# liznerski/eoe

Measured on AMD Instinct MI355X. Metric: train images/sec, CLIP ViT-B/32 + HSC, 224x224, higher is better.
Workload: dtype fp16; 1 GPU; CLIP ViT-B/32 (12 layers) + Linear(512,256) + HSC, full fine-tune, Adam lr 1e-4 wd 1e-3, 224x224, 128 normal + 128 OE images per GPU per step; global_batch=256, parallelism=dp1, launch=eager, weight-gradient launches on a side stream under the dgrad chain, arithmetic=16-bit MFMA operands, fp32 accumulate

## Files before the change

### eoe_amd/_build.py

```python
import fcntl
import hashlib
import os
import shutil
import subprocess
import sys

HERE = os.path.dirname(os.path.abspath(__file__))
CSRC = os.path.join(HERE, "csrc")
INCLUDE = os.path.join(os.path.dirname(HERE), "include")
LIB = os.path.join(HERE, "libeoe_hip.so")
OBJDIR = os.path.join(HERE, "build")
SOURCES = ["api.cpp", "gemm.hip", "gemm_tn.hip", "elementwise.hip", "attention.hip", "conv.hip", "cbam.hip", "augment.hip",
           "vit.cpp", "parity.hip", "gemm256.hip", "comm.cpp", "gemm_tn256.hip", "gemm_w8.hip", "probe.hip",
           "msm.hip", "sharpen.hip", "clip_text.hip", "clip_text_driver.cpp", "normstats.hip", "evolve.hip", "curves.hip"]
CFLAGS = ["--offload-arch=gfx950", "-O3", "-std=c++17", "-fPIC", "-Wno-unused-value"]
EXTRA_CFLAGS = {"gemm_w8.hip": ["-mllvm", "-amdgpu-spill-vgpr-to-agpr=0"]}
LDFLAGS = ["--offload-arch=gfx950", "-shared", "-fPIC", "-Wl,--no-undefined"]


def hipcc_path():
    for cand in (shutil.which("hipcc"), "/opt/rocm/bin/hipcc"):
        if cand and os.path.exists(cand):
            return cand
    return None


def _sha(*chunks) -> str:
    h = hashlib.sha256()
    for c in chunks:
        h.update(c if isinstance(c, bytes) else str(c).encode())
        h.update(b"\0")
    return h.hexdigest()


def _read(path) -> bytes:
    with open(path, "rb") as f:
        return f.read()


def _headers_digest() -> str:
    hs = sorted(os.path.join(CSRC, f) for f in os.listdir(CSRC) if f.endswith((".h", ".hpp", ".inc")))
    hs += sorted(os.path.join(INCLUDE, f) for f in os.listdir(INCLUDE) if f.endswith(".h"))
    return _sha(*[_read(h) for h in hs])


def _flags(src: str = ""):
    return CFLAGS + EXTRA_CFLAGS.get(src, []) + (["-DEOE_AB"] if os.environ.get("EOE_AB") else []) + os.environ.get("EOE_CFLAGS", "").split()
# ... 88 lines not shown
```

### eoe_amd/_lib.py

```python
import ctypes as C
import os
import re

import torch

from . import _build

ABI_VERSION = 5
EOE_F16, EOE_BF16, EOE_F32 = 1, 2, 3
EOE_RESIZE_BILINEAR, EOE_RESIZE_BICUBIC = 2, 3
EOE_MSM_LPF, EOE_MSM_HPF, EOE_MSM_BLUR = 1, 2, 3
EOE_MSM_FORM_NONE, EOE_MSM_FORM_DENSE, EOE_MSM_FORM_RANK = 0, 1, 2
EOE_GCN_L1, EOE_GCN_L2 = 1, 2
EOE_COMM_I64, EOE_COMM_ID_BYTES, EOE_COMM_ALGO_RING, EOE_COMM_ALGO_RS_AG = 8, 128, 0, 1
EPI_NONE, EPI_GELU, EPI_RESIDUAL, EPI_GELU_BWD = 0, 1, 2, 3
ADAM_CHUNK, ADAM_GROUPS = 8192, 4
CHUNK_FP16 = 0x100
EOE_Y16 = 0x100

_vp, _i32, _i64, _f32, _sz = C.c_void_p, C.c_int32, C.c_int64, C.c_float, C.c_size_t


class ConvGeometry(C.Structure):
    _fields_ = [("n", _i32), ("H", _i32), ("W", _i32), ("C", _i32), ("kh", _i32), ("kw", _i32), ("stride", _i32), ("pad", _i32),
# ... 95 lines not shown
    _fields_ = [("f", VitBlockFwdArgs), ("dx_out", _vp), ("dx_in", _vp),
                ("g_ln1_g", _vp), ("g_ln1_b", _vp), ("g_ln2_g", _vp), ("g_ln2_b", _vp),
                ("g_b_in", _vp), ("g_b_out", _vp), ("g_b_fc", _vp), ("g_b_proj", _vp),
                ("g_w_in", _vp), ("g_w_out", _vp), ("g_w_fc", _vp), ("g_w_proj", _vp),
                ("accumulate", _i32),
                ("d16_a", _vp), ("d16_b", _vp), ("d16_c", _vp), ("dh", _vp), ("dqkv", _vp), ("dx_mid", _vp), ("red_scratch", _vp),
                ("tn_workspace", _vp), ("tn_workspace_bytes", _i64),
                ("next_d16", _vp), ("in_d16", _vp), ("in_red_scratch", _vp), ("async_wgrad", _i32), ("red_table", C.POINTER(RedTable))]


ALLREDUCE_FN = C.CFUNCTYPE(C.c_int, C.c_void_p, C.c_void_p, C.c_int64, C.c_int, C.c_void_p)

SIGNATURES = {
    "eoe_abi_version": [],
    "eoe_struct_size": [C.c_int],
    "eoe_last_error": [],
    "eoe_vit_side_join": [_vp],
    "eoe_red_table_flush": [C.POINTER(RedTable), _vp],
    "eoe_gemm_nt": [C.POINTER(GemmArgs), _vp],
    "eoe_gemm_tn": [C.POINTER(GemmArgs), _vp],
    "eoe_gemm_tn_grouped": [C.POINTER(GemmArgs), C.c_int, _vp],
    "eoe_cast_transpose": [_vp, _vp, _vp, C.c_int, C.c_int, C.c_int, _vp],
    "eoe_cast_transpose_multi": [_vp, C.c_int, C.c_int, _vp],
    "eoe_conv_pack_weight_multi": [_vp, C.c_int, C.c_int, _vp],
    "eoe_patchify": [_vp, _vp, _vp, _vp, C.c_int, C.c_int, C.c_int, C.c_int, _vp],
    "eoe_embed_lnpre_fwd": [_vp] * 8 + [C.c_int, C.c_int, C.c_int, _f32, _vp],
    "eoe_embed_lnpre_bwd": [_vp] * 10 + [C.c_int, C.c_int, C.c_int, C.c_int, _vp],
    "eoe_layernorm_fwd": [_vp, C.c_int, _vp, _vp, _vp, _vp, C.c_int, C.c_int, _f32, C.c_int, C.c_int, _vp],
    "eoe_layernorm_bwd": [_vp, C.c_int, _vp, C.c_int, _vp, _vp, _vp, _vp, C.c_int, _vp, _vp, _vp, _vp, _vp, C.c_int,
                          C.c_int, C.c_int, _vp],
    "eoe_linear_small_fwd": [_vp, _vp, _vp, _vp, C.c_int, C.c_int, C.c_int, _vp],
    "eoe_linear_small_bwd": [_vp, _vp, _vp, _vp, _vp, _vp, C.c_int, C.c_int, C.c_int, C.c_int, _vp],
    "eoe_zero_multi": [C.POINTER(_vp), C.POINTER(C.c_int), C.c_int, _vp],
    "eoe_cast_colsum": [_vp, _vp, _vp, _vp, C.c_int, C.c_int, C.c_int, C.c_int, _vp],
    "eoe_colsum": [_vp, C.c_int, _vp, C.c_int, C.c_int, C.c_int, C.c_int, _vp],
    "eoe_colsum_det": [_vp, C.c_int, _vp, _vp, C.c_int, C.c_int, C.c_int, _vp],
    "eoe_cast": [_vp, _vp, _sz, C.c_int, _vp],
    "eoe_attn_fwd": [_vp, _vp, C.c_int, C.c_int, C.c_int, C.c_int, _vp],
    "eoe_attn_bwd": [_vp, _vp, _vp, _vp, _vp, C.c_int, C.c_int, C.c_int, C.c_int, _vp],
    "eoe_attn_causal_fwd": [_vp, _vp, C.c_int, C.c_int, C.c_int, C.c_int, _vp],
    "eoe_clip_token_embed": [_vp, C.c_int, _vp, _vp, _vp, C.c_int, C.c_int, C.c_int, C.c_int, _vp],
    "eoe_clip_eot_ln": [_vp, _vp, C.c_int, _vp, _vp, _vp, C.c_int, C.c_int, C.c_int, _f32, C.c_int, _vp],
    "eoe_clip_text_fwd": [C.POINTER(ClipTextFwdArgs), _vp],
    "eoe_hsc_fwd": [_vp, _vp, _i64, _vp, _vp, _vp, _vp, C.c_int, C.c_int, _f32, _vp],
    "eoe_hsc_bwd": [_vp, _vp, _i64, _vp, _vp, _vp, C.c_int, C.c_int, _f32, C.c_int, _vp],
    "eoe_hsc_score": [_vp, _vp, C.c_int, C.c_int, _vp],
    "eoe_bce_fwd": [_vp, _vp, _i64, _vp, _vp, _vp, C.c_int, _f32, _vp],
    "eoe_bce_bwd": [_vp, _vp, _vp, _vp, C.c_int, _f32, _vp],
    "eoe_adam_tiles": [_vp, _vp, _vp, _vp, _vp, C.c_int, C.POINTER(AdamScalars), _f32, _f32, _f32, _f32, C.c_int, _vp, _vp],
    "eoe_adam_multi": [_vp, _vp, _vp, _vp, _vp, C.c_int, C.POINTER(AdamScalars), _f32, _f32, _f32, _f32, _vp, C.c_int,
                       _vp, _vp],
    "eoe_grads_nonfinite": [_vp, _vp, C.c_int, _vp, C.c_int, C.c_int, _vp],
    "eoe_vit_block_fwd": [C.POINTER(VitBlockFwdArgs), _vp],
    "eoe_vit_block_bwd": [C.POINTER(VitBlockBwdArgs), _vp],
    "eoe_im2col": [_vp, C.c_int, _vp, _vp, _vp] + [C.c_int] * 10 + [_vp],
    "eoe_col2im": [_vp, _vp] + [C.c_int] * 11 + [_vp],
    "eoe_conv_pack_weight": [_vp, _vp, _vp, _vp] + [C.c_int] * 7 + [_vp],
    "eoe_conv_unpack_wgrad": [_vp, _vp] + [C.c_int] * 8 + [_vp],
    "eoe_stem_pack_image": [_vp, _vp, _vp, _vp] + [C.c_int] * 8 + [_vp],
    "eoe_stem_pack_weight": [_vp, _vp] + [C.c_int] * 4 + [_vp],
    "eoe_stem_unpack_wgrad": [_vp, _vp] + [C.c_int] * 3 + [_vp],
    "eoe_bn_stats": [_vp, _vp, _vp, _vp, _vp, _vp, C.c_int, C.c_int, _f32, _f32, C.c_int, _vp],
    "eoe_bn_stats_partials": [_vp, C.c_int, _vp, _vp, _vp, _vp, _vp, C.c_int, C.c_int, _f32, _f32, _vp],
    "eoe_bn_act_pool_fwd": [_vp, _vp, _vp, _vp, _vp, _vp, C.c_int, C.c_int, C.c_int, C.c_int, C.c_int, C.c_int, C.c_int, _f32,
                            C.c_int, _vp],
    "eoe_colsum_f32": [_vp, _vp, _vp, C.c_int, C.c_int, C.c_int, _vp],
# ... 146 lines not shown
```

### eoe_amd/csrc/elementwise.hip

```cpp
#include "common.h"

namespace {

template <typename T>
__global__ __launch_bounds__(256) void cast_kernel(const float* __restrict__ src, T* __restrict__ dst, size_t n) {
    size_t i = ((size_t)blockIdx.x * blockDim.x + threadIdx.x) * 4;
    const size_t stride = (size_t)gridDim.x * blockDim.x * 4;
    for (; i + 3 < n; i += stride) {
        f32x4 v = *(const f32x4*)(src + i);
        *(u32x2*)(dst + i) = pack4<T>(v[0], v[1], v[2], v[3]);
    }
    if (blockIdx.x == 0 && threadIdx.x < (n & 3)) {
        size_t j = (n & ~(size_t)3) + threadIdx.x;
        dst[j] = (T)src[j];
    }
}

template <typename T>
__global__ __launch_bounds__(256) void cast_transpose_kernel(const float* __restrict__ src, T* __restrict__ dst, T* __restrict__ dst_t,
                                      int rows, int cols) {
    __shared__ float tile[64][65];
    const int c0 = blockIdx.x * 64, r0 = blockIdx.y * 64;
    const int tx = threadIdx.x & 63, ty = threadIdx.x >> 6;
    for (int r = ty; r < 64; r += 4) {
// ... 108 lines not shown
    const int c = blockIdx.x * 256 + cg * 4;
    float a[4] = {0.f, 0.f, 0.f, 0.f};
    if (c < cols) {
        for (int r = blockIdx.y * 4 + rl; r < rows; r += gridDim.y * 4) {
            const f32x4 v = *(const f32x4*)(x + (size_t)r * cols + c);
            *(u32x2*)(dst + (size_t)r * cols + c) = pack4<T>(v[0], v[1], v[2], v[3]);
#pragma unroll
            for (int k = 0; k < 4; ++k) a[k] += v[k];
        }
    }
#pragma unroll
    for (int k = 0; k < 4; ++k) red[rl][cg * 4 + k] = a[k];
    __syncthreads();
    const int cc = blockIdx.x * 256 + threadIdx.x;
    if (cc >= cols) return;
    const float t = (red[0][threadIdx.x] + red[1][threadIdx.x]) + (red[2][threadIdx.x] + red[3][threadIdx.x]);
    if (part) part[eoe_part_index(cc, blockIdx.y, gridDim.y, cols, blocked)] = t;
    else atomicAdd(out + cc, t);
}

struct ZeroArgs { float* p[EOE_ZERO_MAX]; int n[EOE_ZERO_MAX]; int count; };
__global__ __launch_bounds__(256) void zero_multi_kernel(ZeroArgs a) {
    const int b = blockIdx.y;
    if (b >= a.count) return;
    float* p = a.p[b];
    const int n = a.n[b];
    if ((((uintptr_t)p) & 15) == 0) {
        const int n4 = n >> 2;
        for (int i = blockIdx.x * blockDim.x + threadIdx.x; i < n4; i += gridDim.x * blockDim.x) ((f32x4*)p)[i] = (f32x4){0.f, 0.f, 0.f, 0.f};
        for (int i = (n4 << 2) + blockIdx.x * blockDim.x + threadIdx.x; i < n; i += gridDim.x * blockDim.x) p[i] = 0.f;
    } else {
        for (int i = blockIdx.x * blockDim.x + threadIdx.x; i < n; i += gridDim.x * blockDim.x) p[i] = 0.f;
    }
}

template <typename T>
__global__ __launch_bounds__(256) void patchify_kernel(const float* __restrict__ x, const float* __restrict__ mean,
                                const float* __restrict__ stdv, T* __restrict__ out, int res, int p) {
    const int g = res / p;
    const int n = blockIdx.x / g, py = blockIdx.x % g;
    const int kdim = 3 * p * p;
    float mu[3] = {0.f, 0.f, 0.f}, is[3] = {1.f, 1.f, 1.f};
    if (mean) {
#pragma unroll
        for (int c = 0; c < 3; ++c) { mu[c] = mean[c]; is[c] = 1.0f / stdv[c]; }
    }
    const int rq_row = res >> 2;
    const int nq = 3 * p * rq_row;
    const int sq = 256 / rq_row, rq = 256 - sq * rq_row;
    int i = threadIdx.x;
    int c = i / (p * rq_row), rem = i - c * (p * rq_row);
    int ky = rem / rq_row, xq = rem - ky * rq_row;
    const float* img = x + (size_t)n * 3 * res * res + (size_t)py * p * res;
    T* orow = out + (size_t)(n * g + py) * g * kdim;
    constexpr int U = 4;
    while (i < nq) {
        f32x4 v[U];
        int cc[U], oo[U];
#pragma unroll
        for (int u = 0; u < U; ++u) {
            const bool ok = i < nq;
            const int xx = xq * 4;
            v[u] = *(const f32x4*)(img + (ok ? ((size_t)c * res + ky) * res + xx : (size_t)0));
            const int px = xx / p, kx = xx - px * p;
            cc[u] = c;
            oo[u] = ok ? px * kdim + c * p * p + ky * p + kx : -1;
// ... 1243 lines not shown
    }
    if (dw) {
        if (!accumulate) {
            if (hipMemsetAsync(dw, 0, (size_t)N * K * sizeof(float), s) != hipSuccess ||
                (db && hipMemsetAsync(db, 0, (size_t)N * sizeof(float), s) != hipSuccess))
                return eoe_set_error(EOE_ERR_LAUNCH, "linear_small_bwd: memset failed");
        }
        int gy = cdiv(M, 32);
        if (gy > 64) gy = 64;
        hipLaunchKernelGGL(linear_small_dw_kernel, dim3(cdiv(K, 256), gy), dim3(256), 0, s, x, dy, dw, db, M, N, K);
        EOE_CHECK_LAUNCH("linear_small_dw");
    }
    return 0;
}

extern "C" int eoe_zero_multi(float* const* ptrs, const int* counts, int n, void* stream) {
    EOE_CHECK_ARG(ptrs && counts && n >= 1 && n <= EOE_ZERO_MAX, "zero_multi: n %d not in [1, %d]", n, EOE_ZERO_MAX);
    ZeroArgs a;
    int mx = 0;
    for (int i = 0; i < n; ++i) {
        EOE_CHECK_ARG(ptrs[i] && counts[i] >= 0, "zero_multi: bad buffer %d", i);
        a.p[i] = ptrs[i]; a.n[i] = counts[i];
        if (counts[i] > mx) mx = counts[i];
    }
    a.count = n;
    int gx = cdiv(mx, 1024);
    if (gx > 2048) gx = 2048;
    if (gx < 1) gx = 1;
    hipLaunchKernelGGL(zero_multi_kernel, dim3(gx, n), dim3(256), 0, (hipStream_t)stream, a);
    EOE_CHECK_LAUNCH("zero_multi");
    return 0;
}

extern "C" int eoe_cast_colsum(const float* x, void* dst, float* out, float* scratch, int rows, int cols, int dtype, int accumulate,
                               void* stream) {
    EOE_CHECK_ARG(x && dst && out && rows > 0 && cols > 0, "cast_colsum: bad args");
    EOE_CHECK_ARG(cols % 4 == 0, "cast_colsum: cols must be a multiple of 4");
    ProfScope ps("cast_colsum", 0, 6.0 * rows * cols, stream);
    int gy = cdiv(rows, 4 * 8);
    if (gy > EOE_CAST_COLSUM_PARTIALS) gy = EOE_CAST_COLSUM_PARTIALS;
    const bool deferred_mode = scratch && eoe_tls_defer;
    const int blocked = (cols & 63) == 0;
    if (!accumulate && !deferred_mode) {
        if (hipMemsetAsync(out, 0, (size_t)cols * sizeof(float), (hipStream_t)stream) != hipSuccess)
            return eoe_set_error(EOE_ERR_LAUNCH, "cast_colsum: memset failed");
    }
    DISPATCH_T(dtype, hipLaunchKernelGGL((cast_colsum_kernel<T>), dim3(cdiv(cols, 256), gy), dim3(256), 0,
                                         (hipStream_t)stream, x, (T*)dst, out, scratch, rows, cols, blocked));
    EOE_CHECK_LAUNCH("cast_colsum");
    if (scratch) EOE_TRY(eoe_finish_reduce(scratch, gy, cols, cols, out, nullptr, nullptr, blocked, stream));
    return 0;
}

extern "C" int eoe_hsc_fwd(const float* f, const int64_t* labels, int64_t nominal_label, float* loss, float* scores,
                           float* dists, float* losses, int n, int d, float inv_count, void* stream) {
    EOE_CHECK_ARG(f && labels && n > 0 && d > 0, "hsc_fwd: bad args");
    EOE_CHECK_ARG(!loss || losses, "hsc_fwd: the loss needs the per-sample `losses` buffer");
    hipLaunchKernelGGL(hsc_rows_kernel, dim3(cdiv(n, 4)), dim3(256), 0, (hipStream_t)stream, f, labels, nominal_label,
                       scores, dists, losses, n, d);
    EOE_CHECK_LAUNCH("hsc_rows");
    if (loss) {
        hipLaunchKernelGGL(sum_scale_kernel, dim3(1), dim3(256), 0, (hipStream_t)stream, losses, loss, n, inv_count);
        EOE_CHECK_LAUNCH("hsc_sum");
    }
    return 0;
}
// ... 200 lines not shown
```

### eoe_amd/csrc/gemm.hip

```cpp
#include "gemm_common.h"
#include <stdlib.h>
#include <map>
#include <mutex>
#include <type_traits>

unsigned long long* g_stamp_buf = nullptr;
extern int g_tn_flags;
extern int g_vit_side_stream;
extern int g_attn_flags;
extern int g_tn256_launches;
extern int g_parity_flags;
int eoe_launch_nt256(const void* gemm_p, int dtype, int epi, int mi, hipStream_t s);
bool eoe_w8_applies(const void* gemm_p, int epi);
int eoe_launch_w8(const void* gemm_p, int dtype, int epi, hipStream_t s);
bool eoe_w8_streamk(const void* gemm_p);

namespace {
extern int g_nt_flags;


template <typename T, int EPI, int NI, int FLAGS, int GATHER = 0>
__global__ __launch_bounds__(512, 2) void gemm_nt_kernel(GemmP p) {
    extern __shared__ __attribute__((aligned(16))) char smem[];
    const int tid = threadIdx.x, lane = tid & 63, wave = tid >> 6;
    constexpr int BNI = 32 * NI;
    const int tiles_n = (p.N + BNI - 1) / BNI;
    const int total_tiles = tiles_n * ((p.M + BM - 1) / BM);
    const int G = gridDim.x;
    const int my_tiles = (total_tiles - (int)blockIdx.x + G - 1) / G;
    const int nk = p.K / BK;
    const int iters = my_tiles * nk;

    __amdgpu_buffer_rsrc_t ra = make_rsrc(p.A, p.bytesA);
    __amdgpu_buffer_rsrc_t rb = make_rsrc(p.B, p.bytesB);

    unsigned offA[4], offB[2];
    int gh[4], gw[4];
    int gw3[4];
    int g_ky = 0, g_kx = 0, g_c0 = 0;
    int st_tile = 0, st_kt = 0, st_slot = 0;
    auto tile_origin = [&](int seq, int& m0, int& n0) {
        const int r = xcd_remap((int)blockIdx.x + seq * G, total_tiles);
        m0 = (r / tiles_n) * BM;
        n0 = (r % tiles_n) * BNI;
    };
    auto set_offsets = [&](int t) {
        int m0, n0;
// ... 641 lines not shown
    EOE_CHECK_LAUNCH("gemm_nt128");
    return finish_colsum(p, epi, MI, s);
}

template <typename T>
int launch_nt128w(const GemmP& p, int epi, hipStream_t s) {
    const int tiles = cdiv(p.M, 160) * cdiv(p.N, 256);
#define EOE_NT128W_CASE(E)                                                                  \
    case E:                                                                                 \
        { static bool once = (hipFuncSetAttribute((const void*)gemm_nt128w_kernel<T, E>, hipFuncAttributeMaxDynamicSharedMemorySize, SMEMW_BYTES), true); (void)once; } \
        hipLaunchKernelGGL((gemm_nt128w_kernel<T, E>), dim3(tiles), dim3(256), SMEMW_BYTES, s, p); \
        break;
    switch (epi) {
        EOE_NT128W_CASE(EOE_EPI_NONE)
        EOE_NT128W_CASE(EOE_EPI_GELU)
        EOE_NT128W_CASE(EOE_EPI_RESIDUAL)
        EOE_NT128W_CASE(EOE_EPI_GELU_BWD)
        default: return eoe_set_error(EOE_ERR_ARG, "gemm_nt: unknown epilogue %d", epi);
    }
#undef EOE_NT128W_CASE
    EOE_CHECK_LAUNCH("gemm_nt128w");
    return finish_colsum(p, epi, 5, s);
}

template <typename T>
int launch_nt128_auto(const GemmP& p, int epi, hipStream_t s) {
    const int slots = 2 * num_cus();
    const long t4 = (long)cdiv(p.M, 128) * cdiv(p.N, 128), t5 = (long)cdiv(p.M, 160) * cdiv(p.N, 128);
    const long c4 = (t4 + slots - 1) / slots * 128, c5 = (t5 + slots - 1) / slots * 160;
    const bool five = (g_nt_flags & 32) || (!(g_nt_flags & 16) && c5 <= c4);
    return five ? launch_nt128<T, 5>(p, epi, s) : launch_nt128<T, 4>(p, epi, s);
}

template <typename T>
__global__ __launch_bounds__(256) void nt_splitk_finish_kernel(const float* __restrict__ part, int S, int M, int N, float alpha,
                                                               const float* __restrict__ bias, const float* __restrict__ res, int ldres,
                                                               void* __restrict__ C, int ldc, int out_f32) {
    const int nq = N / 4;
    const int i = blockIdx.x * blockDim.x + threadIdx.x;
    if (i >= M * nq) return;
    const int m = i / nq, n = (i - m * nq) * 4;
    f32x4 v = *(const f32x4*)(part + (size_t)m * N + n);
    for (int s2 = 1; s2 < S; ++s2) v += *(const f32x4*)(part + ((size_t)s2 * M + m) * N + n);
    v *= alpha;
    if (bias) v += *(const f32x4*)(bias + n);
    if (res) v += *(const f32x4*)(res + (size_t)m * ldres + n);
    if (out_f32) *(f32x4*)((float*)C + (size_t)m * ldc + n) = v;
    else *(u32x2*)((T*)C + (size_t)m * ldc + n) = pack4<T>(v[0], v[1], v[2], v[3]);
}

template <typename T>
int launch_nt128_splitk(const GemmP& p, int epi, hipStream_t s) {
    const int nk = p.K / BK;
    if ((g_nt_flags & 8192) || !p.split_k || p.M > 1024 || nk < 24 || (epi != EOE_EPI_NONE && epi != EOE_EPI_RESIDUAL) || p.colsum || p.colsum_sq || p.accumulate ||
        (p.N & 15) || (p.ldc & 3) || (epi == EOE_EPI_RESIDUAL && (p.ldaux & 3)))
        return -1;
    int S = 8;
    while (S > 1 && (nk % S) != 0) S >>= 1;
    if (S < 2 || nk / S < 3) return -1;
    float* part = p.sk_part;
    if (!part || (size_t)S * p.M * p.N > (size_t)2 * num_cus() * 65536) return -1;
    GemmP q = p;
    q.C = part; q.ldc = p.N; q.out_f32 = 1; q.bias = nullptr; q.aux = nullptr; q.alpha = 1.0f;
    const int tiles = cdiv(p.M, 128) * cdiv(p.N, 128);
    { static bool once = (hipFuncSetAttribute((const void*)gemm_nt128_kernel<T, EOE_EPI_NONE, 4>, hipFuncAttributeMaxDynamicSharedMemorySize, smem128_bytes(4)), true); (void)once; }
    hipLaunchKernelGGL((gemm_nt128_kernel<T, EOE_EPI_NONE, 4>), dim3(tiles, S), dim3(256), smem128_bytes(4), s, q);
    EOE_CHECK_LAUNCH("gemm_nt128 (split k)");
    hipLaunchKernelGGL((nt_splitk_finish_kernel<T>), dim3(cdiv(p.M * (p.N / 4), 256)), dim3(256), 0, s, (const float*)part, S, p.M, p.N, p.alpha,
                       p.bias, epi == EOE_EPI_RESIDUAL ? (const float*)p.aux : nullptr, p.ldaux, p.C, p.ldc, p.out_f32);
    EOE_CHECK_LAUNCH("nt_splitk_finish");
    return 0;
}


int g_nt_flags = EOE_NT_DEFAULT_FLAGS;

template <typename T, int NI, int FLAGS>
int launch_nt_f(const GemmP& p, int epi, int grid, hipStream_t s) {
#define EOE_NT_CASE(E)                                                                      \
    case E:                                                                                 \
        { static bool once = (hipFuncSetAttribute((const void*)gemm_nt_kernel<T, E, NI, FLAGS>, hipFuncAttributeMaxDynamicSharedMemorySize, SMEM_BYTES), true); (void)once; } \
        hipLaunchKernelGGL((gemm_nt_kernel<T, E, NI, FLAGS>), dim3(grid), dim3(512), SMEM_BYTES, s, p); \
        break;
    switch (epi) {
        EOE_NT_CASE(EOE_EPI_NONE)
        EOE_NT_CASE(EOE_EPI_GELU)
        EOE_NT_CASE(EOE_EPI_RESIDUAL)
        EOE_NT_CASE(EOE_EPI_GELU_BWD)
        default: return eoe_set_error(EOE_ERR_ARG, "gemm_nt: unknown epilogue %d", epi);
    }
#undef EOE_NT_CASE
    EOE_CHECK_LAUNCH("gemm_nt");
    return finish_colsum(p, epi, 4, s);
}

template <typename T, int NI, int GATHER>
int launch_nt_conv(const GemmP& p, int grid, hipStream_t s) {
    static bool once = (hipFuncSetAttribute((const void*)gemm_nt_kernel<T, EOE_EPI_NONE, NI, EOE_NT_DEFAULT_FLAGS, GATHER>,
                                            hipFuncAttributeMaxDynamicSharedMemorySize, SMEM_BYTES), true);
    (void)once;
    hipLaunchKernelGGL((gemm_nt_kernel<T, EOE_EPI_NONE, NI, EOE_NT_DEFAULT_FLAGS, GATHER>), dim3(grid), dim3(512), SMEM_BYTES, s, p);
    EOE_CHECK_LAUNCH("gemm_nt");
    return finish_colsum(p, EOE_EPI_NONE, 4, s);
}

template <typename T, int NI>
int launch_nt_ni(const GemmP& p, int epi, int grid, hipStream_t s) {
#ifdef EOE_AB
    switch (g_nt_flags & 3) {
        case 0: return launch_nt_f<T, NI, 0>(p, epi, grid, s);
        case 1: return launch_nt_f<T, NI, 1>(p, epi, grid, s);
        case 2: return launch_nt_f<T, NI, 2>(p, epi, grid, s);
        default: return launch_nt_f<T, NI, 3>(p, epi, grid, s);
    }
#else
    return launch_nt_f<T, NI, EOE_NT_DEFAULT_FLAGS>(p, epi, grid, s);
#endif
}

template <typename T>
int launch_nt(const GemmP& p, int epi, int gather, hipStream_t s) {
    const int ncu = num_cus();
    if (epi == EOE_EPI_NONE && p.N <= 64 && (gather == 0 || gather == 1 || gather == 2) && !(g_nt_flags & 64)) {
        const int rc = gather == 2 ? launch_nt64<T, 2>(p, s) : (gather ? launch_nt64<T, 1>(p, s) : launch_nt64<T, 0>(p, s));
        return rc ? rc : finish_colsum(p, EOE_EPI_NONE, 4, s);
    }
    if (gather == 1 && epi == EOE_EPI_NONE && p.N >= 128 && !(g_nt_flags & 2048)) {
        const int slots = 2 * ncu;
        const long t4 = (long)cdiv(p.M, 128) * cdiv(p.N, 128), t5 = (long)cdiv(p.M, 160) * cdiv(p.N, 128);
        const long c4 = (t4 + slots - 1) / slots * 128, c5 = (t5 + slots - 1) / slots * 160;
        if (!p.colsum_sq && c5 < c4) return launch_nt128_gather<T, 5>(p, s);
        return launch_nt128_gather<T, 4>(p, s);
    }
    if (gather || (epi == EOE_EPI_NONE && p.N <= 64)) {
        const bool narrow = p.N <= 64;
        const int tiles = cdiv(p.M, BM) * cdiv(p.N, narrow ? 64 : 128);
        const int grid = tiles < ncu ? tiles : ncu;
        if (gather == 2) return narrow ? launch_nt_conv<T, 2, 2>(p, grid, s) : launch_nt_conv<T, 4, 2>(p, grid, s);
        if (gather == 3) return narrow ? launch_nt_conv<T, 2, 3>(p, grid, s) : launch_nt_conv<T, 4, 3>(p, grid, s);
        if (gather) return narrow ? launch_nt_conv<T, 2, 1>(p, grid, s) : launch_nt_conv<T, 4, 1>(p, grid, s);
        return launch_nt_conv<T, 2, 0>(p, grid, s);
    }
    if ((g_nt_flags & (128 | 256)) && epilogue_direct_ok(p, epi))
        return eoe_launch_nt256(&p, std::is_same<T, f16_t>::value ? EOE_F16 : EOE_BF16, epi, (g_nt_flags & 256) ? 8 : 5, s);
    const bool big = p.K >= 4096 && p.N >= 2048;
    if (gather == 0 && p.split_k) {
        const int rc = launch_nt128_splitk<T>(p, epi, s);
        if (rc >= 0) return rc;
    }
    if (!(g_nt_flags & (131072 | 4 | 8 | 512)) && gather == 0 && p.M >= 2048 && eoe_w8_applies(&p, epi)) {
        const long tiles = (long)cdiv(p.M, 256) * (p.N / 256);
        if ((g_nt_flags & 262144) || eoe_w8_streamk(&p) || tiles * 100 >= ((tiles + ncu - 1) / ncu) * ncu * 85) 
            return eoe_launch_w8(&p, std::is_same<T, f16_t>::value ? EOE_F16 : EOE_BF16, epi, s);
    }
    if (!(g_nt_flags & (4096 | 4 | 8 | 512)) && gather == 0 && !p.colsum_sq && (p.N % 256) == 0 && p.N >= 2048 && (p.K % 32) == 0 && p.M >= 2048) {
        const long tiles = (long)cdiv(p.M, 160) * (p.N / 256), slots = 2L * ncu;
        if (tiles * 10 >= ((tiles + slots - 1) / slots) * slots * 9) return launch_nt128w<T>(p, epi, s);
    }
    const bool gelu_wide = epi == EOE_EPI_GELU && p.N >= 2048 && p.K <= 1024 && !(g_nt_flags & 1024);
    if (((g_nt_flags & 512) || gelu_wide) && !(g_nt_flags & (4 | 8)) && epilogue_direct_ok(p, epi) && p.M >= 2048 && p.N >= 512) {
        const int nk = p.K / BK;
        long best = 0;
        int mi_best = 5;
        for (int mi : {5, 8}) {
            const long tiles = (long)cdiv(p.M, 32 * mi) * cdiv(p.N, 256);
            const long cost = ((tiles + ncu - 1) / ncu) * ((long)mi * (nk + 2) + 30);
            if (!best || cost < best) { best = cost; mi_best = mi; }
        }
        return eoe_launch_nt256(&p, std::is_same<T, f16_t>::value ? EOE_F16 : EOE_BF16, epi, mi_best, s);
    }
    if (big && !(g_nt_flags & (4 | 8)) && epilogue_direct_ok(p, epi) && p.M >= 2048)
        return eoe_launch_nt256(&p, std::is_same<T, f16_t>::value ? EOE_F16 : EOE_BF16, epi, 8, s);
    if (!p.colsum_sq && ((g_nt_flags & 8) || (!big && !(g_nt_flags & 4)))) return launch_nt128_auto<T>(p, epi, s);
    const int t4 = cdiv(p.M, BM) * cdiv(p.N, 128), t3 = cdiv(p.M, BM) * cdiv(p.N, 96);
    const int c4 = cdiv(t4, ncu) * 4, c3 = cdiv(t3, ncu) * 3;
    const int force = (g_nt_flags >> 4) & 7;
    const bool use3 = force ? (force == 3) : (c3 * 10 <= c4 * 9);
    const int tiles = use3 ? t3 : t4;
    const int grid = tiles < ncu ? tiles : ncu;
    return use3 ? launch_nt_ni<T, 3>(p, epi, grid, s) : launch_nt_ni<T, 4>(p, epi, grid, s);
// ... 135 lines not shown
```

### eoe_amd/csrc/vit.cpp

```cpp
#include "common.h"
#include <mutex>
#include <stdlib.h>

#define TRY(expr)                   \
    do {                            \
        int rc__ = (expr);          \
        if (rc__ != 0) return rc__; \
    } while (0)

extern int g_tn_flags;
bool eoe_tn_streamk_would_run(const eoe_gemm_args* args, int count, void* stream);
int eoe_red_table_append(eoe_red_table* t, EoeRedJobs* jobs, void* stream);
int g_vit_side_stream = 1;

namespace {

struct SideStream {
    hipStream_t s = nullptr;
    hipEvent_t fork = nullptr, join = nullptr, wgrad_done[2] = {nullptr, nullptr};
    bool ok = false;
    unsigned seq = 0;
    bool recorded[2] = {false, false};
};
SideStream* side_stream(hipStream_t main) {
// ... 96 lines not shown
    } guard(b->red_scratch ? &jobs : nullptr);
    float* red_fc = b->red_scratch;
    float* red_ln2 = red_fc ? red_fc + (size_t)((M + 63) / 64) * H : nullptr;
    float* red_attn = red_fc ? red_ln2 + EOE_LN_SCRATCH(D) : nullptr;
    float* red_ln1 = red_fc ? red_attn + (size_t)a->n * 3 * D : nullptr;
    float* red_cast = red_fc ? red_ln1 + EOE_LN_SCRATCH(D) : nullptr;
    eoe_gemm_args g, w[4];
    const bool handed = !cls && b->in_d16 && b->in_red_scratch && b->red_scratch && b->in_red_scratch != b->red_scratch;
    const void* dy_proj = handed ? b->in_d16 : b->d16_a;
    if (handed) {
        const float* in_ln1 = b->in_red_scratch + (size_t)((M + 63) / 64) * H + EOE_LN_SCRATCH(D) + (size_t)a->n * 3 * D;
        int rows = (M + 7) / 8;
        if (rows > EOE_LN_PARTIALS) rows = EOE_LN_PARTIALS;
        if (!eoe_defer_reduce(in_ln1, rows, 3 * D, D, nullptr, nullptr, b->g_b_proj, 1))
            return eoe_set_error(EOE_ERR_ARG, "vit_block_bwd: could not queue the handed-over column sums");
    } else {
        TRY(eoe_cast_colsum(b->dx_out, b->d16_a, b->g_b_proj, red_cast, Mo, D, dt, 1, stream));
    }
    g = gemm(a, dy_proj, a->w_proj_t, b->dh, nullptr, Mo, H, D, D, D, H, dt);
    g.epilogue = EOE_EPI_GELU_BWD; g.aux = a->hpre; g.ldaux = H;
    if (b->red_scratch) {
        g.colsum = b->g_b_fc; g.workspace = red_fc; g.workspace_bytes = (int64_t)EOE_NT_COLSUM_WORKSPACE_BYTES(Mo, H);
        TRY(eoe_gemm_nt(&g, stream));
    } else {
        TRY(eoe_gemm_nt(&g, stream));
        TRY(eoe_colsum(b->dh, H, b->g_b_fc, Mo, H, dt, 1, stream));
    }
    g = gemm(a, b->dh, a->w_fc_t, b->d16_b, nullptr, Mo, D, H, H, H, D, dt);
    g.split_k = cls ? 1 : 0;
    TRY(eoe_gemm_nt(&g, stream));
    float* dx_mid_o = cls ? (float*)((char*)b->d16_a + (((size_t)Mo * D * 2 + 255) & ~(size_t)255)) : b->dx_mid;
    TRY(eoe_layernorm_bwd(b->d16_b, 0, a->x_mid, D, a->stats2, a->ln2_g, b->dx_out, dx_mid_o, D, b->d16_c, b->g_ln2_g,
                          b->g_ln2_b, b->g_b_out, red_ln2, Mo, D, dt, stream));
    if (cls) {
        if (hipMemsetAsync(b->dx_mid, 0, (size_t)M * D * sizeof(float), s) != hipSuccess ||
            hipMemcpy2DAsync(b->dx_mid, (size_t)ldrow * sizeof(float), dx_mid_o, (size_t)D * sizeof(float), (size_t)D * sizeof(float), Mo,
                             hipMemcpyDeviceToDevice, s) != hipSuccess ||
            hipMemsetAsync(b->d16_b, 0, (size_t)M * D * 2, s) != hipSuccess)
            return eoe_set_error(EOE_ERR_LAUNCH, "vit_block_bwd: zero-fill / scatter of the class-token rows failed");
    }
    g = gemm(a, b->d16_c, a->w_out_t, b->d16_b, nullptr, Mo, D, D, D, D, ldrow, dt);
    TRY(eoe_gemm_nt(&g, stream));
    TRY(eoe_attn_bwd(a->qkv, b->d16_b, b->dqkv, red_attn ? b->g_b_in : nullptr, red_attn, a->n, a->L, a->heads, dt, stream));
    g = gemm(a, b->dqkv, a->w_in_t, b->d16_b, nullptr, M, D, 3 * D, 3 * D, 3 * D, D, dt);
    TRY(eoe_gemm_nt(&g, stream));
    if (!b->red_scratch) TRY(eoe_colsum(b->dqkv, 3 * D, b->g_b_in, M, 3 * D, dt, 1, stream));
    w[0] = gemm(b->dh, a->xn2, b->g_w_fc, nullptr, H, D, Mo, H, D, D, dt);
    w[1] = gemm(dy_proj, a->hact, b->g_w_proj, nullptr, D, H, Mo, D, H, H, dt);
    w[2] = gemm(b->dqkv, a->xn1, b->g_w_in, nullptr, 3 * D, D, M, 3 * D, D, D, dt);
    w[3] = gemm(b->d16_c, a->att, b->g_w_out, nullptr, D, D, Mo, D, ldrow, D, dt);
    for (int i = 0; i < 4; ++i) { w[i].out_f32 = 1; w[i].accumulate = acc; }
    w[0].workspace = b->tn_workspace; w[0].workspace_bytes = b->tn_workspace ? b->tn_workspace_bytes : 0;
    eoe_gemm_args wc[3] = {w[0], w[1], w[3]};
    w[2].workspace = cls ? w[0].workspace : nullptr; w[2].workspace_bytes = cls ? w[0].workspace_bytes : 0;
    auto launch_wgrads = [&](void* st) -> int {
        if (!cls) return eoe_gemm_tn_grouped(w, 4, st);
        TRY(eoe_gemm_tn_grouped(wc, 3, st));
        return eoe_gemm_tn_grouped(&w[2], 1, st);
    };
    const bool streamk = !cls && eoe_tn_streamk_would_run(w, 4, stream);
    SideStream* ss = (g_vit_side_stream == 2 || (g_vit_side_stream && (!streamk || b->async_wgrad))) && b->red_scratch ? side_stream(s) : nullptr;
    if (ss && b->async_wgrad) {
        const unsigned e_prev = (ss->seq + 1) & 1, e_old = ss->seq & 1;
        if (ss->recorded[e_old]) {
            if (hipStreamWaitEvent(s, ss->wgrad_done[e_old], 0) != hipSuccess) return eoe_set_error(EOE_ERR_LAUNCH, "vit_block_bwd: stream wait failed");
            ss->recorded[e_old] = false;
        }
        if (b->async_wgrad < 2 && ss->recorded[e_prev]) {
            if (hipStreamWaitEvent(s, ss->wgrad_done[e_prev], 0) != hipSuccess) return eoe_set_error(EOE_ERR_LAUNCH, "vit_block_bwd: stream wait failed");
            ss->recorded[e_prev] = false;
        }
        if (hipEventRecord(ss->fork, s) != hipSuccess || hipStreamWaitEvent(ss->s, ss->fork, 0) != hipSuccess)
            return eoe_set_error(EOE_ERR_LAUNCH, "vit_block_bwd: fork failed");
// ... 40 lines not shown
```

### include/eoe_hip.h

```cpp
#ifndef EOE_HIP_H
#define EOE_HIP_H

#include <stddef.h>
#include <stdint.h>

#ifdef __cplusplus
extern "C" {
#endif

#define EOE_ABI_VERSION 5

enum { EOE_OK = 0, EOE_ERR_ARG = 1, EOE_ERR_LAUNCH = 2, EOE_ERR_UNSUPPORTED = 3 };
enum { EOE_F16 = 1, EOE_BF16 = 2, EOE_F32 = 3  };

int eoe_abi_version(void);
int eoe_struct_size(int which);
const char* eoe_last_error(void);

enum {
    EOE_EPI_NONE = 0,
    EOE_EPI_GELU = 1,
    EOE_EPI_RESIDUAL = 2,
    EOE_EPI_GELU_BWD = 3
};
// ... 52 lines not shown
int eoe_patchify(const float* x, const float* mean, const float* std, void* out, int n, int res, int patch,
                 int dtype, void* stream);

int eoe_embed_lnpre_fwd(const float* tok, const float* cls, const float* pos, const float* gamma,
                        const float* beta, float* x0, float* y, float* stats, int n, int L, int D, float eps,
                        void* stream);
int eoe_embed_lnpre_bwd(const float* dy, const float* x0, const float* stats, const float* gamma, void* dtok,
                        float* dcls, float* dpos, float* dgamma, float* dbeta, float* scratch, int n, int L, int D, int dtype,
                        void* stream);

int eoe_layernorm_fwd(const float* x, int ldx, const float* gamma, const float* beta, void* y, float* stats,
                      int rows, int D, float eps, int dtype, int out_f32, void* stream);
#define EOE_LN_PARTIALS 512
#define EOE_LN_SCRATCH(D) ((size_t)EOE_LN_PARTIALS * 3 * (D))
int eoe_layernorm_bwd(const void* dy, int dy_f32, const float* x, int ldx, const float* stats,
                      const float* gamma, const float* dres, float* dx_out, int ld_out, void* dx16,
                      float* dgamma, float* dbeta, float* dxsum, float* red_scratch, int rows, int D, int dtype,
                      void* stream);

int eoe_colsum(const void* x, int ldx, float* out, int rows, int cols, int dtype, int accumulate, void* stream);
#define EOE_COLSUM_PARTIALS 256
int eoe_colsum_det(const void* x, int ldx, float* out, float* scratch, int rows, int cols, int dtype, void* stream);

#define EOE_CAST_COLSUM_PARTIALS 256
int eoe_cast_colsum(const float* x, void* dst, float* out, float* scratch, int rows, int cols, int dtype, int accumulate, void* stream);

int eoe_linear_small_fwd(const float* x, const float* w, const float* bias, float* y, int M, int N, int K, void* stream);
int eoe_linear_small_bwd(const float* x, const float* w, const float* dy, float* dx, float* dw, float* db, int M, int N,
                         int K, int accumulate, void* stream);

#define EOE_ZERO_MAX 12
int eoe_zero_multi(float* const* ptrs, const int* counts, int n, void* stream);

int eoe_cast(const float* src, void* dst, size_t n, int dtype, void* stream);

int eoe_attn_fwd(const void* qkv, void* out, int n, int L, int heads, int dtype, void* stream);
int eoe_attn_bwd(const void* qkv, const void* dout, void* dqkv, float* dbias, float* bias_scratch, int n, int L, int heads,
                 int dtype, void* stream);

int eoe_attn_causal_fwd(const void* qkv, void* out, int n, int L, int heads, int dtype, void* stream);
int eoe_clip_token_embed(const void* tok, int tok_i64, const float* token_embedding, const float* positional_embedding, float* out, int n,
                         int L, int D, int vocab, void* stream);
int eoe_clip_eot_ln(const float* x, const void* tok, int tok_i64, const float* gamma, const float* beta, void* y, int n, int L, int D,
                    float eps, int dtype, void* stream);
typedef struct {
    int32_t n, L, D, heads, layers, vocab, embed_dim, dtype;
    float eps;
    int32_t tok_i64;
    const void* tokens;
    const float* token_embedding;
    const float* positional_embedding;
    const float* const* ln1_g; const float* const* ln1_b; const float* const* ln2_g; const float* const* ln2_b;
    const float* const* b_in; const float* const* b_out; const float* const* b_fc; const float* const* b_proj;
    const void* const* w_in; const void* const* w_out; const void* const* w_fc; const void* const* w_proj;
    const float *lnf_g, *lnf_b;
    const void* proj_t;
    float *x0, *x1;
    void *xn, *qkv, *att, *hact;
    float* stats;
    void* eot16;
    float* out;
    void* nt_sk_workspace;
    int64_t nt_sk_workspace_bytes;
} eoe_clip_text_fwd_args;
int eoe_clip_text_fwd(const eoe_clip_text_fwd_args* args, void* stream);

// ... 339 lines not shown
```

Before: 25570 images/sec.

## Add small-M rows GEMM kernel and fuse class-token scatter and zero-fill

Measured after the change: 25690 images/sec, median of 6. About the same (+0.5%).

```diff
diff --git a/eoe_amd/_build.py b/eoe_amd/_build.py
--- a/eoe_amd/_build.py
+++ b/eoe_amd/_build.py
@@ -12,7 +12,7 @@
 OBJDIR = os.path.join(HERE, "build")
 SOURCES = ["api.cpp", "gemm.hip", "gemm_tn.hip", "elementwise.hip", "attention.hip", "conv.hip", "cbam.hip", "augment.hip",
            "vit.cpp", "parity.hip", "gemm256.hip", "comm.cpp", "gemm_tn256.hip", "gemm_w8.hip", "probe.hip",
-           "msm.hip", "sharpen.hip", "clip_text.hip", "clip_text_driver.cpp", "normstats.hip", "evolve.hip", "curves.hip"]
+           "msm.hip", "sharpen.hip", "clip_text.hip", "clip_text_driver.cpp", "normstats.hip", "evolve.hip", "curves.hip", "gemm_rows.hip"]
 CFLAGS = ["--offload-arch=gfx950", "-O3", "-std=c++17", "-fPIC", "-Wno-unused-value"]
 EXTRA_CFLAGS = {"gemm_w8.hip": ["-mllvm", "-amdgpu-spill-vgpr-to-agpr=0"]}
 LDFLAGS = ["--offload-arch=gfx950", "-shared", "-fPIC", "-Wl,--no-undefined"]
diff --git a/eoe_amd/_lib.py b/eoe_amd/_lib.py
--- a/eoe_amd/_lib.py
+++ b/eoe_amd/_lib.py
@@ -151,6 +151,7 @@
     "eoe_linear_small_fwd": [_vp, _vp, _vp, _vp, C.c_int, C.c_int, C.c_int, _vp],
     "eoe_linear_small_bwd": [_vp, _vp, _vp, _vp, _vp, _vp, C.c_int, C.c_int, C.c_int, C.c_int, _vp],
     "eoe_zero_multi": [C.POINTER(_vp), C.POINTER(C.c_int), C.c_int, _vp],
+    "eoe_cls_scatter_fill": [_vp, _vp, _vp, C.c_int, C.c_int, C.c_int, _vp],
     "eoe_cast_colsum": [_vp, _vp, _vp, _vp, C.c_int, C.c_int, C.c_int, C.c_int, _vp],
     "eoe_colsum": [_vp, C.c_int, _vp, C.c_int, C.c_int, C.c_int, C.c_int, _vp],
     "eoe_colsum_det": [_vp, C.c_int, _vp, _vp, C.c_int, C.c_int, C.c_int, _vp],
diff --git a/eoe_amd/csrc/elementwise.hip b/eoe_amd/csrc/elementwise.hip
--- a/eoe_amd/csrc/elementwise.hip
+++ b/eoe_amd/csrc/elementwise.hip
@@ -164,6 +164,20 @@
     } else {
         for (int i = blockIdx.x * blockDim.x + threadIdx.x; i < n; i += gridDim.x * blockDim.x) p[i] = 0.f;
     }
+}
+
+__global__ __launch_bounds__(256) void cls_scatter_fill_kernel(f32x4* __restrict__ dx_mid, const f32x4* __restrict__ dx_cls,
+                                                               u32x4* __restrict__ d16, unsigned n4, unsigned n8, FDiv q, FDiv L) {
+    const unsigned stride = gridDim.x * blockDim.x, t = blockIdx.x * blockDim.x + threadIdx.x;
+    for (unsigned i = t; i < n4; i += stride) {
+        unsigned row, c, img, l;
+        q.divmod(i, row, c);
+        L.divmod(row, img, l);
+        f32x4 v = {0.f, 0.f, 0.f, 0.f};
+        if (l == 0) v = dx_cls[img * q.d + c];
+        dx_mid[i] = v;
+    }
+    for (unsigned i = t; i < n8; i += stride) d16[i] = (u32x4){0u, 0u, 0u, 0u};
 }
 
 template <typename T>
@@ -1473,6 +1487,19 @@
     return 0;
 }
 
+extern "C" int eoe_cls_scatter_fill(float* dx_mid, const float* dx_cls, void* d16, int n, int L, int D, void* stream) {
+    EOE_CHECK_ARG(dx_mid && dx_cls && d16 && n > 0 && L > 0 && D > 0 && (D % 8) == 0, "cls_scatter_fill: bad args (D must be a multiple of 8)");
+    EOE_CHECK_ARG(((((uintptr_t)dx_mid) | ((uintptr_t)dx_cls) | ((uintptr_t)d16)) & 15) == 0, "cls_scatter_fill: buffers must be 16-byte aligned");
+    const long long n4 = (long long)n * L * (D / 4);
+    EOE_CHECK_ARG(n4 < 0x7fffffffll, "cls_scatter_fill: %d x %d x %d is too large", n, L, D);
+    int gx = (int)((n4 + 255) / 256);
+    if (gx > 2048) gx = 2048;
+    hipLaunchKernelGGL(cls_scatter_fill_kernel, dim3(gx), dim3(256), 0, (hipStream_t)stream, (f32x4*)dx_mid, (const f32x4*)dx_cls, (u32x4*)d16,
+                       (unsigned)n4, (unsigned)(n4 / 2), FDiv((unsigned)(D / 4)), FDiv((unsigned)L));
+    EOE_CHECK_LAUNCH("cls_scatter_fill");
+    return 0;
+}
+
 extern "C" int eoe_cast_colsum(const float* x, void* dst, float* out, float* scratch, int rows, int cols, int dtype, int accumulate,
                                void* stream) {
     EOE_CHECK_ARG(x && dst && out && rows > 0 && cols > 0, "cast_colsum: bad args");
diff --git a/eoe_amd/csrc/gemm.hip b/eoe_amd/csrc/gemm.hip
--- a/eoe_amd/csrc/gemm.hip
+++ b/eoe_amd/csrc/gemm.hip
@@ -1,4 +1,5 @@
 #include "gemm_common.h"
+#include "gemm_rows_plan.h"
 #include <stdlib.h>
 #include <map>
 #include <mutex>
@@ -13,6 +14,7 @@
 int eoe_launch_nt256(const void* gemm_p, int dtype, int epi, int mi, hipStream_t s);
 bool eoe_w8_applies(const void* gemm_p, int epi);
 int eoe_launch_w8(const void* gemm_p, int dtype, int epi, hipStream_t s);
+int eoe_launch_nt_rows(const void* gemm_p, int dtype, int epi, int splits, hipStream_t s);
 bool eoe_w8_streamk(const void* gemm_p);
 
 namespace {
@@ -720,6 +722,14 @@
     return five ? launch_nt128<T, 5>(p, epi, s) : launch_nt128<T, 4>(p, epi, s);
 }
 
+static EoeNtPlanIn plan_in(const GemmP& p, int epi, int gather) {
+    EoeNtPlanIn q;
+    q.M = p.M; q.N = p.N; q.K = p.K; q.epi = epi; q.split_k = p.split_k; q.flags = g_nt_flags; q.gather = gather;
+    q.colsum = p.colsum != nullptr; q.colsum_sq = p.colsum_sq; q.accumulate = p.accumulate; q.ldc = p.ldc; q.ldaux = p.ldaux;
+    q.part_floats = p.sk_part ? (long long)2 * num_cus() * 65536 : 0;
+    return q;
+}
+
 template <typename T>
 __global__ __launch_bounds__(256) void nt_splitk_finish_kernel(const float* __restrict__ part, int S, int M, int N, float alpha,
                                                                const float* __restrict__ bias, const float* __restrict__ res, int ldres,
@@ -738,22 +748,20 @@
 }
 
 template <typename T>
-int launch_nt128_splitk(const GemmP& p, int epi, hipStream_t s) {
-    const int nk = p.K / BK;
-    if ((g_nt_flags & 8192) || !p.split_k || p.M > 1024 || nk < 24 || (epi != EOE_EPI_NONE && epi != EOE_EPI_RESIDUAL) || p.colsum || p.colsum_sq || p.accumulate ||
-        (p.N & 15) || (p.ldc & 3) || (epi == EOE_EPI_RESIDUAL && (p.ldaux & 3)))
-        return -1;
-    int S = 8;
-    while (S > 1 && (nk % S) != 0) S >>= 1;
-    if (S < 2 || nk / S < 3) return -1;
+int launch_nt128_splitk(const GemmP& p, int epi, bool rows, hipStream_t s) {
+    const int S = eoe_nt_splits(plan_in(p, epi, 0));
+    if (S < 2) return -1;
     float* part = p.sk_part;
-    if (!part || (size_t)S * p.M * p.N > (size_t)2 * num_cus() * 65536) return -1;
     GemmP q = p;
     q.C = part; q.ldc = p.N; q.out_f32 = 1; q.bias = nullptr; q.aux = nullptr; q.alpha = 1.0f;
-    const int tiles = cdiv(p.M, 128) * cdiv(p.N, 128);
-    { static bool once = (hipFuncSetAttribute((const void*)gemm_nt128_kernel<T, EOE_EPI_NONE, 4>, hipFuncAttributeMaxDynamicSharedMemorySize, smem128_bytes(4)), true); (void)once; }
-    hipLaunchKernelGGL((gemm_nt128_kernel<T, EOE_EPI_NONE, 4>), dim3(tiles, S), dim3(256), smem128_bytes(4), s, q);
-    EOE_CHECK_LAUNCH("gemm_nt128 (split k)");
+    if (rows) {
+        EOE_TRY(eoe_launch_nt_rows(&q, std::is_same<T, f16_t>::value ? EOE_F16 : EOE_BF16, EOE_EPI_NONE, S, s));
+    } else {
+        const int tiles = cdiv(p.M, 128) * cdiv(p.N, 128);
+        { static bool once = (hipFuncSetAttribute((const void*)gemm_nt128_kernel<T, EOE_EPI_NONE, 4>, hipFuncAttributeMaxDynamicSharedMemorySize, smem128_bytes(4)), true); (void)once; }
+        hipLaunchKernelGGL((gemm_nt128_kernel<T, EOE_EPI_NONE, 4>), dim3(tiles, S), dim3(256), smem128_bytes(4), s, q);
+        EOE_CHECK_LAUNCH("gemm_nt128 (split k)");
+    }
     hipLaunchKernelGGL((nt_splitk_finish_kernel<T>), dim3(cdiv(p.M * (p.N / 4), 256)), dim3(256), 0, s, (const float*)part, S, p.M, p.N, p.alpha,
                        p.bias, epi == EOE_EPI_RESIDUAL ? (const float*)p.aux : nullptr, p.ldaux, p.C, p.ldc, p.out_f32);
     EOE_CHECK_LAUNCH("nt_splitk_finish");
@@ -809,6 +817,10 @@
 template <typename T>
 int launch_nt(const GemmP& p, int epi, int gather, hipStream_t s) {
     const int ncu = num_cus();
+    if (eoe_nt_rows_applies(plan_in(p, epi, gather))) {
+        const int rc = launch_nt128_splitk<T>(p, epi, true, s);
+        return rc >= 0 ? rc : eoe_launch_nt_rows(&p, std::is_same<T, f16_t>::value ? EOE_F16 : EOE_BF16, epi, 1, s);
+    }
     if (epi == EOE_EPI_NONE && p.N <= 64 && (gather == 0 || gather == 1 || gather == 2) && !(g_nt_flags & 64)) {
         const int rc = gather == 2 ? launch_nt64<T, 2>(p, s) : (gather ? launch_nt64<T, 1>(p, s) : launch_nt64<T, 0>(p, s));
         return rc ? rc : finish_colsum(p, EOE_EPI_NONE, 4, s);
@@ -833,7 +845,7 @@
         return eoe_launch_nt256(&p, std::is_same<T, f16_t>::value ? EOE_F16 : EOE_BF16, epi, (g_nt_flags & 256) ? 8 : 5, s);
     const bool big = p.K >= 4096 && p.N >= 2048;
     if (gather == 0 && p.split_k) {
-        const int rc = launch_nt128_splitk<T>(p, epi, s);
+        const int rc = launch_nt128_splitk<T>(p, epi, false, s);
         if (rc >= 0) return rc;
     }
     if (!(g_nt_flags & (131072 | 4 | 8 | 512)) && gather == 0 && p.M >= 2048 && eoe_w8_applies(&p, epi)) {
diff --git a/eoe_amd/csrc/gemm_rows.hip b/eoe_amd/csrc/gemm_rows.hip
--- /dev/null
+++ b/eoe_amd/csrc/gemm_rows.hip
@@ -0,0 +1,114 @@
+#include "gemm_common.h"
+
+namespace {
+
+constexpr int ROWS_TILE = 64;
+constexpr int ROWS_SLOTS = 8;
+constexpr int ROWS_HALF_BYTES = ROWS_TILE * BK * 2;
+constexpr int ROWS_SLOT_BYTES = 2 * ROWS_HALF_BYTES;
+constexpr int ROWS_SMEM_BYTES = ROWS_SLOTS * ROWS_SLOT_BYTES;
+static_assert(ROWS_SLOTS == 8, "the counted wait below is 4 * (ROWS_SLOTS - 2) = 24 and the slot index is masked with 7");
+
+template <typename T, int EPI>
+__global__ __launch_bounds__(256, 1) void gemm_rows_kernel(GemmP p) {
+    extern __shared__ __attribute__((aligned(16))) char smem[];
+    constexpr int MI = 4, NI = 1;
+    const int tid = threadIdx.x, lane = tid & 63, wave = tid >> 6;
+    const int tiles_n = (p.N + ROWS_TILE - 1) / ROWS_TILE;
+    const int mt = (int)blockIdx.x / tiles_n, nt = (int)blockIdx.x - mt * tiles_n;
+    const int m0 = mt * ROWS_TILE, n0 = nt * ROWS_TILE;
+    const int nk = (p.K / BK) / (int)gridDim.y;
+    const unsigned kbase = (unsigned)blockIdx.y * (unsigned)nk * (BK * 2u);
+
+    __amdgpu_buffer_rsrc_t ra = make_rsrc(p.A, p.bytesA);
+    __amdgpu_buffer_rsrc_t rb = make_rsrc(p.B, p.bytesB);
+    unsigned offA[2], offB[2];
+#pragma unroll
+    for (int j = 0; j < 2; ++j) {
+        const int row = (wave * 2 + j) * 8 + (lane >> 3);
+        const int c = (lane & 7) ^ ((row >> 1) & 7);
+        offA[j] = (m0 + row < p.M) ? (unsigned)(((size_t)(m0 + row) * p.lda + c * 8) * 2) : EOE_OOB;
+        offB[j] = (n0 + row < p.N) ? (unsigned)(((size_t)(n0 + row) * p.ldb + c * 8) * 2) : EOE_OOB;
+    }
+#define EOE_STAGE_ROWS(kt)                                                                                                   \
+    do {                                                                                                                     \
+        char* sa_ = smem + ((kt) & (ROWS_SLOTS - 1)) * ROWS_SLOT_BYTES;                                                      \
+        char* sb_ = sa_ + ROWS_HALF_BYTES;                                                                                   \
+        const bool on_ = (kt) < nk;                                                                                          \
+        const unsigned k0_ = kbase + (unsigned)(kt) * (BK * 2u);                                                             \
+        _Pragma("unroll") for (int j = 0; j < 2; ++j)                                                                        \
+            __builtin_amdgcn_raw_ptr_buffer_load_lds(ra, (lds_void_t*)(sa_ + (wave * 2 + j) * 1024), 16,                     \
+                                                     on_ ? offA[j] + k0_ : EOE_OOB, 0, 0, 0);                                 \
+        _Pragma("unroll") for (int j = 0; j < 2; ++j)                                                                        \
+            __builtin_amdgcn_raw_ptr_buffer_load_lds(rb, (lds_void_t*)(sb_ + (wave * 2 + j) * 1024), 16,                     \
+                                                     on_ ? offB[j] + k0_ : EOE_OOB, 0, 0, 0);                                 \
+    } while (0)
+
+    const int lr = lane & 15, lg = lane >> 4;
+    const int sw = (lr >> 1) & 7;
+    const int fragA = lr * 128, fragB = ROWS_HALF_BYTES + (wave * 16 + lr) * 128;
+    const int ch0 = ((0 + lg) ^ sw) * 16, ch1 = ((4 + lg) ^ sw) * 16;
+    typedef typename T16<T>::v8 V8;
+
+    f32x4 acc[MI][NI];
+#pragma unroll
+    for (int i = 0; i < MI; ++i) acc[i][0] = (f32x4){0.f, 0.f, 0.f, 0.f};
+
+#pragma unroll
+    for (int s = 0; s < ROWS_SLOTS - 1; ++s) EOE_STAGE_ROWS(s);
+    for (int kt = 0; kt < nk; ++kt) {
+        EOE_WAIT_VM(24);
+        EOE_WAIT_LGKM0();
+        __builtin_amdgcn_s_barrier();
+        EOE_STAGE_ROWS(kt + ROWS_SLOTS - 1);
+        const char* sc = smem + (kt & (ROWS_SLOTS - 1)) * ROWS_SLOT_BYTES;
+        V8 xa0[MI], xa1[MI], wb0, wb1;
+#pragma unroll
+        for (int i = 0; i < MI; ++i) xa0[i] = *(const V8*)(sc + fragA + i * 2048 + ch0);
+        wb0 = *(const V8*)(sc + fragB + ch0);
+#pragma unroll
+        for (int i = 0; i < MI; ++i) xa1[i] = *(const V8*)(sc + fragA + i * 2048 + ch1);
+        wb1 = *(const V8*)(sc + fragB + ch1);
+#pragma unroll
+        for (int mi = 0; mi < MI; ++mi) acc[mi][0] = T16<T>::mfma16(wb0, xa0[mi], acc[mi][0]);
+#pragma unroll
+        for (int mi = 0; mi < MI; ++mi) acc[mi][0] = T16<T>::mfma16(wb1, xa1[mi], acc[mi][0]);
+    }
+#undef EOE_STAGE_ROWS
+    EOE_WAIT_VM(0);
+    EOE_WAIT_LGKM0();
+    __builtin_amdgcn_s_barrier();
+    GemmP ep;
+    load_epilogue_args(ep, p);
+    if (gridDim.y > 1) ep.C = (char*)ep.C + (size_t)blockIdx.y * (size_t)ep.M * ep.ldc * sizeof(float);
+    epilogue<T, EPI, NI, MI>(ep, acc, m0, n0 + wave * 16, lane, smem + wave * 4096);
+}
+
+template <typename T>
+int launch_rows(const GemmP& p, int epi, int splits, hipStream_t s) {
+    const dim3 grid(cdiv(p.M, ROWS_TILE) * cdiv(p.N, ROWS_TILE), splits);
+#define EOE_ROWS_CASE(E)                                                                    \
+    case E:                                                                                 \
+        { static bool once = (hipFuncSetAttribute((const void*)gemm_rows_kernel<T, E>, hipFuncAttributeMaxDynamicSharedMemorySize, ROWS_SMEM_BYTES), true); (void)once; } \
+        hipLaunchKernelGGL((gemm_rows_kernel<T, E>), grid, dim3(256), ROWS_SMEM_BYTES, s, p); \
+        break;
+    switch (epi) {
+        EOE_ROWS_CASE(EOE_EPI_NONE)
+        EOE_ROWS_CASE(EOE_EPI_GELU)
+        EOE_ROWS_CASE(EOE_EPI_RESIDUAL)
+        EOE_ROWS_CASE(EOE_EPI_GELU_BWD)
+        default: return eoe_set_error(EOE_ERR_ARG, "gemm_nt: unknown epilogue %d", epi);
+    }
+#undef EOE_ROWS_CASE
+    EOE_CHECK_LAUNCH("gemm_rows");
+    return finish_colsum(p, epi, 4, s);
+}
+
+}
+
+int eoe_launch_nt_rows(const void* gemm_p, int dtype, int epi, int splits, hipStream_t s) {
+    const GemmP& p = *(const GemmP*)gemm_p;
+    if (p.M > 8 * ROWS_TILE || splits < 1 || (p.K / BK) % splits != 0 || p.colsum_sq)
+        return eoe_set_error(EOE_ERR_ARG, "gemm_rows: M = %d, %d k-ranges over K = %d: not a problem of the small-M kernel", p.M, splits, p.K);
+    return dtype == EOE_F16 ? launch_rows<f16_t>(p, epi, splits, s) : launch_rows<bf16_t>(p, epi, splits, s);
+}
diff --git a/eoe_amd/csrc/gemm_rows_plan.h b/eoe_amd/csrc/gemm_rows_plan.h
--- /dev/null
+++ b/eoe_amd/csrc/gemm_rows_plan.h
@@ -0,0 +1,30 @@
+#pragma once
+#include "../../include/eoe_hip.h"
+
+#define EOE_NT_ROWS_MAX_M 512
+#define EOE_NT_FLAG_ROWS_OFF 16777216
+#define EOE_NT_FLAGS_FORCED (4 | 8 | 16 | 32 | 64 | 128 | 256 | 512)
+
+struct EoeNtPlanIn {
+    int M, N, K, epi, split_k, flags, gather;
+    int colsum, colsum_sq, accumulate;
+    int ldc, ldaux;
+    long long part_floats;
+};
+
+static inline int eoe_nt_splits(const EoeNtPlanIn& q) {
+    const int nk = q.K / 64;
+    if ((q.flags & 8192) || !q.split_k || q.gather || q.M > 1024 || nk < 24 || (q.epi != EOE_EPI_NONE && q.epi != EOE_EPI_RESIDUAL) || q.colsum ||
+        q.colsum_sq || q.accumulate || (q.N & 15) || (q.ldc & 3) || (q.epi == EOE_EPI_RESIDUAL && (q.ldaux & 3)))
+        return 0;
+    if (q.epi == EOE_EPI_NONE && q.N <= 64) return 0;
+    int S = 8;
+    while (S > 1 && (nk % S) != 0) S >>= 1;
+    if (S < 2 || nk / S < 3) return 0;
+    if ((long long)S * q.M * q.N > q.part_floats) return 0;
+    return S;
+}
+
+static inline bool eoe_nt_rows_applies(const EoeNtPlanIn& q) {
+    return q.gather == 0 && q.M <= EOE_NT_ROWS_MAX_M && !q.colsum_sq && !(q.flags & (EOE_NT_FLAG_ROWS_OFF | EOE_NT_FLAGS_FORCED));
+}
diff --git a/eoe_amd/csrc/vit.cpp b/eoe_amd/csrc/vit.cpp
--- a/eoe_amd/csrc/vit.cpp
+++ b/eoe_amd/csrc/vit.cpp
@@ -152,13 +152,7 @@
     float* dx_mid_o = cls ? (float*)((char*)b->d16_a + (((size_t)Mo * D * 2 + 255) & ~(size_t)255)) : b->dx_mid;
     TRY(eoe_layernorm_bwd(b->d16_b, 0, a->x_mid, D, a->stats2, a->ln2_g, b->dx_out, dx_mid_o, D, b->d16_c, b->g_ln2_g,
                           b->g_ln2_b, b->g_b_out, red_ln2, Mo, D, dt, stream));
-    if (cls) {
-        if (hipMemsetAsync(b->dx_mid, 0, (size_t)M * D * sizeof(float), s) != hipSuccess ||
-            hipMemcpy2DAsync(b->dx_mid, (size_t)ldrow * sizeof(float), dx_mid_o, (size_t)D * sizeof(float), (size_t)D * sizeof(float), Mo,
-                             hipMemcpyDeviceToDevice, s) != hipSuccess ||
-            hipMemsetAsync(b->d16_b, 0, (size_t)M * D * 2, s) != hipSuccess)
-            return eoe_set_error(EOE_ERR_LAUNCH, "vit_block_bwd: zero-fill / scatter of the class-token rows failed");
-    }
+    if (cls) TRY(eoe_cls_scatter_fill(b->dx_mid, dx_mid_o, b->d16_b, a->n, a->L, D, stream));
     g = gemm(a, b->d16_c, a->w_out_t, b->d16_b, nullptr, Mo, D, D, D, D, ldrow, dt);
     TRY(eoe_gemm_nt(&g, stream));
     TRY(eoe_attn_bwd(a->qkv, b->d16_b, b->dqkv, red_attn ? b->g_b_in : nullptr, red_attn, a->n, a->L, a->heads, dt, stream));
diff --git a/include/eoe_hip.h b/include/eoe_hip.h
--- a/include/eoe_hip.h
+++ b/include/eoe_hip.h
@@ -108,6 +108,8 @@
 #define EOE_ZERO_MAX 12
 int eoe_zero_multi(float* const* ptrs, const int* counts, int n, void* stream);
 
+int eoe_cls_scatter_fill(float* dx_mid, const float* dx_cls, void* d16, int n, int L, int D, void* stream);
+
 int eoe_cast(const float* src, void* dst, size_t n, int dtype, void* stream);
 
 int eoe_attn_fwd(const void* qkv, void* out, int n, int L, int heads, int dtype, void* stream);
```
